# gongaa/SlidingWindowDecoder

Hardware: AMD Instinct MI355X
Metric: sliding windows decoded/s, [[144,12,12]] BB p=0.003 (higher is better)
Workload: dtype f64

## Files before the change

### slidingwindowdecoder_amd/csrc/swd_osdw_kernel.h

```cpp
#pragma once
#include <type_traits>
#include <hip/hip_runtime.h>
#include <stdint.h>

#include "swd.h"
#include "swd_graph.h"

#define SWD_DMAX 10

#ifndef SWD_OSDW_TUNED
#define SWD_OSDW_TUNED 0
#endif
#ifndef SWD_TUNED_NT
#define SWD_TUNED_NT 256
#endif
#define SWD_P16(NT) (SWD_OSDW_TUNED && (NT) <= SWD_TUNED_NT)
#ifndef SWD_POST_DEPTH2
#define SWD_POST_DEPTH2 0
#endif
#ifndef SWD_POST_SORTED
#define SWD_POST_SORTED 3
#endif
#ifndef SWD_POST_KGP
#define SWD_POST_KGP 0
// ... 155 lines not shown
template <int NT>
__device__ __forceinline__ bool block_any(bool p, Lds &s) {
    constexpr int NW = NT / 64;
    const int par = (s.fpar++) & 1;
    unsigned long long b = __ballot(p);
    if ((threadIdx.x & 63) == 0) s.flags[par * 16 + (threadIdx.x >> 6)] = (b != 0ull);
    __syncthreads();
    int r = 0;
#pragma unroll
    for (int w = 0; w < NW; ++w) r |= s.flags[par * 16 + w];
#ifdef SWD_NO_SCALAR_ANY
    return r != 0;
#else
    return __builtin_amdgcn_readfirstlane(r) != 0;
#endif
}

template <int NT>
__device__ __forceinline__ int block_exscan(int x, Lds &s, int &total) {
    constexpr int NW = NT / 64;
    const int lane = threadIdx.x & 63, wave = threadIdx.x >> 6;
    int incl = x;
#pragma unroll
    for (int d = 1; d < 64; d <<= 1) {
        int y = __shfl_up(incl, d, 64);
        if (lane >= d) incl += y;
    }
    int *wsum = s.scal + 8;
    __syncthreads();
    if (lane == 63) wsum[wave] = incl;
    __syncthreads();
    int off = 0, tot = 0;
#pragma unroll
    for (int w = 0; w < NW; ++w) {
        int c = wsum[w];
        if (w < wave) off += c;
        tot += c;
    }
    total = tot;
    return off + incl - x;
}

__device__ __forceinline__ uint64_t f2key(double x) {
    x = x + 0.0;
    uint64_t u = (uint64_t)__double_as_longlong(x);
    return (u >> 63) ? ~u : (u | 0x8000000000000000ull);
}

__device__ __forceinline__ int wave_max(int x) {
#pragma unroll
    for (int d = 32; d > 0; d >>= 1) x = max(x, __shfl_xor(x, d, 64));
    return x;
}

__device__ __forceinline__ void wave_fence() {
    __builtin_amdgcn_fence(__ATOMIC_SEQ_CST, "workgroup");
    __builtin_amdgcn_wave_barrier();
}

template <int VF, int DM, int SH = 0, bool PB = true>
struct VnCacheP {
    static_assert(DM % 2 == 0, "edge offsets are packed in pairs");
    static constexpr bool par_bytes = PB;
    static constexpr int par_shift = (SH == 0 && !PB) ? 2 : 0;
    double llr[VF];
    uint32_t edp[VF][DM / 2];
    __device__ __forceinline__ void set_ed(int i, int k, uint32_t v) { v >>= SH; edp[i][k >> 1] = (k & 1) ? ((edp[i][k >> 1] & 0xFFFFu) | (v << 16)) : ((edp[i][k >> 1] & 0xFFFF0000u) | v); }
    __device__ __forceinline__ void get_ed(int i, uint32_t (&ad)[DM]) const {
#pragma unroll
        for (int k = 0; k < DM; k += 2) {
            uint32_t w = edp[i][k >> 1];
            asm volatile("" : "+v"(w));
            ad[k] = (w & 0xFFFFu) << SH; ad[k + 1] = (w >> 16) << SH;
        }
    }
    uint32_t par[VF][(DM + 1) / 2];
};

__device__ __forceinline__ int swd_slot_far(const SwdGraphDev &g) { return g.E + 1 + (int)(threadIdx.x >> 6); }
template <int NT>
__device__ __forceinline__ int swd_slot_zero(const SwdGraphDev &g) { return g.E + 1 + NT / 64 + (int)(threadIdx.x >> 6); }

template <int NT, int VF, int DM>
struct VnRaw { uint32_t ev[VF][DM]; double llr[VF]; };
template <int NT, int VF, int DM>
__device__ __forceinline__ void vn_cache_issue(const SwdGraphDev &g, const Lds &s, VnRaw<NT, VF, DM> &r) {
    const int n = g.n, D = g.D;
    const uint32_t *et = g.vn_edge;
    const double *lt = g.llr;
#pragma unroll
    for (int i = 0; i < VF; ++i) {
        const int idx = s.vtid + i * NT;
        const int v = (idx < n) ? idx : 0;
        r.llr[i] = (n > 0) ? lt[v] : 0.0;
#pragma unroll
        for (int k = 0; k < DM; ++k) r.ev[i][k] = (n > 0) ? et[max(min(k, D - 1), 0) * n + v] : SWD_PAD_EDGE;
    }
}
template <int NT, int VF, int DM, int SH, bool PB>
__device__ __forceinline__ void vn_cache_pack(const SwdGraphDev &g, const Lds &s, const VnRaw<NT, VF, DM> &r, VnCacheP<VF, DM, SH, PB> &c) {
    const int n = g.n, D = g.D;
    const uint32_t dead = (uint32_t)swd_slot_zero<NT>(g) << 3;
#pragma unroll
    for (int i = 0; i < VF; ++i) {
        const int idx = s.vtid + i * NT;
        const bool valid = idx < n;
        c.llr[i] = valid ? r.llr[i] : 0.0;
#pragma unroll
        for (int k = 0; k < DM; ++k) c.set_ed(i, k, dead);
        constexpr int PS = VnCacheP<VF, DM, SH, PB>::par_shift;
#pragma unroll
        for (int k = 0; k < (DM + 1) / 2; ++k) c.par[i][k] = ((uint32_t)g.m << PS) * 0x10001u;
#pragma unroll
        for (int k = 0; k < DM; ++k) {
            const uint32_t e = r.ev[i][k];
            if (valid && k < D && e != SWD_PAD_EDGE) {
                c.set_ed(i, k, swd_edge_slot(e) << 3);
                c.par[i][k >> 1] = (k & 1) ? ((c.par[i][k >> 1] & 0xFFFFu) | ((swd_edge_lane(e) << PS) << 16))
                                           : ((c.par[i][k >> 1] & 0xFFFF0000u) | (swd_edge_lane(e) << PS));
            }
        }
    }
}

template <int NT, int VF, int DM, bool FULL, bool ALLEDGES = false, bool JPACK = false, int SH, bool PB>
__device__ __forceinline__ void vn_cache_load(const SwdGraphDev &g, Lds &s, int nlive, VnCacheP<VF, DM, SH, PB> &c, uint16_t *remap = nullptr) {
    const int n = g.n, cnt = FULL ? n : nlive;
    const uint32_t dead = (uint32_t)swd_slot_zero<NT>(g) << 3;
    const int D = g.D;
    const uint32_t *et = g.vn_edge;
    const double *lt = g.llr;
    uint32_t ev[VF][DM];
#pragma unroll
    for (int i = 0; i < VF; ++i) {
        const int idx = s.vtid + i * NT;
        const int v = (idx < cnt) ? (FULL ? idx : (int)s.lv[idx]) : 0;
        c.llr[i] = (n > 0) ? lt[v] : 0.0;
#pragma unroll
        for (int k = 0; k < DM; ++k) ev[i][k] = (n > 0) ? et[max(min(k, D - 1), 0) * n + v] : SWD_PAD_EDGE;
    }
#pragma unroll
    for (int i = 0; i < VF; ++i) {
        const int idx = s.vtid + i * NT;
        const bool valid = idx < cnt;
        if (!valid) c.llr[i] = 0.0;
#pragma unroll
        for (int k = 0; k < DM; ++k) c.set_ed(i, k, dead);
        constexpr int PS = VnCacheP<VF, DM, SH, PB>::par_shift;
#pragma unroll
        for (int k = 0; k < (DM + 1) / 2; ++k) c.par[i][k] = ((uint32_t)g.m << PS) * 0x10001u;
#pragma unroll
        for (int k = 0; k < DM; ++k) {
            const uint32_t e = ev[i][k];
            if (valid && k < D && e != SWD_PAD_EDGE) {
                if (FULL || ALLEDGES || s.cn_val[swd_edge_lane(e)] >= 0) {
                    uint32_t slot = swd_edge_slot(e);
                    if (!FULL && remap) { const uint32_t cell = (uint32_t)(k * nlive + idx); remap[slot] = (uint16_t)cell; slot = cell; }
                    c.set_ed(i, k, slot << 3);
                    const uint32_t ph = (swd_edge_lane(e) << PS) | (JPACK ? (swd_edge_j(e) << 10) : 0u);
                    c.par[i][k >> 1] = (k & 1) ? ((c.par[i][k >> 1] & 0xFFFFu) | (ph << 16))
                                               : ((c.par[i][k >> 1] & 0xFFFF0000u) | ph);
                }
            }
        }
    }
}


template <int NT, int VF, int DM, int SH, bool PB>
__device__ __forceinline__ void vn_cache_load_compact(const SwdGraphDev &g, Lds &s, int nlive, VnCacheP<VF, DM, SH, PB> &c, uint16_t *remap, int (&kc)[VF]) {
    const int n = g.n, D = g.D;
    constexpr int PS = VnCacheP<VF, DM, SH, PB>::par_shift;
    const uint32_t dead = (uint32_t)swd_slot_zero<NT>(g) << 3;
    uint32_t ev[VF][DM];
#pragma unroll
    for (int i = 0; i < VF; ++i) {
        const int idx = s.vtid + i * NT;
        const int v = (idx < nlive) ? (int)s.lv[idx] : 0;
        c.llr[i] = (n > 0) ? g.llr[v] : 0.0;
#pragma unroll
// ... 2012 lines not shown
    for (int v = tid; v < n; v += NT) s.hard[v] = 0;
    uint16_t *crows = (uint16_t *)s.scratch;
    bool cols = false;
    constexpr bool kColForm = COLFORM && NT >= 1024 && DM <= 8;
    if constexpr (kColForm) cols = g.wm > 4 && g.wm <= 9 && L.off_oslot >= 0;
    const int nst = min(n, (cols ? L.off_oslot : L.npad * 8) / (DM * 2));
    for (int p = tid; p < nst; p += NT) {
        const int v = idx[p];
        const int deg = g.col_deg[v];
#pragma unroll
        for (int k = 0; k < DM; ++k) crows[p * DM + k] = (k < deg) ? g.vn_row[k * n + v] : (uint16_t)0xFFFF;
    }
    __syncthreads();
    constexpr bool kQuad = QUAD && NT >= 256;
    bool quad = false;
    if constexpr (kQuad) quad = g.wm <= 4 && L.off_oring >= 0;
    if (quad) {
        if constexpr (kQuad) {
            int npiv = 0;
            const int ra = osd0_quad<NT, DM>(g, s, idx, Tc, Sbuf, piv_col, piv_row, synd, crows, nst, &npiv, s.scratch + L.off_oring);
            if (tid == 0) { s.scal[2] = ra; s.scal[3] = npiv; }
        }
    } else if (g.wm <= 4) {
        if (tid < 64) {
            int npiv;
            const int ra = osd0_wave_reg<DM>(g, s, idx, Tc, Sbuf, piv_col, piv_row, synd, crows, nst, &npiv);
            if (tid == 0) { s.scal[2] = ra; s.scal[3] = npiv; }
        }
    } else {
        int npiv = 0, ra = 0;
        bool done = false;
        if constexpr (kColForm) {
            if (cols) { ra = osd0_cols<NT, DM, 9>(g, s, idx, Tc, Sbuf, piv_col, piv_row, synd, crows, nst, &npiv, s.scratch + L.off_oslot); done = true; }
        }
        if constexpr (WIDE && NT == 1024 && DM <= 8) {
            if (g.wm <= 15 && L.off_owide >= 0) {
                ra = osd0_colsw<NT, DM, 15>(g, s, idx, Tc, Sbuf, piv_col, piv_row, synd, crows, nst, &npiv, (char *)s.hard - L.off_hard + L.off_owide, L.owide_ring, L.osd_lds != 0);
                done = true;
            }
        }
        if (!done) ra = osd0_block<NT, DM>(g, s, idx, Tc, Sbuf, piv_col, piv_row, synd, crows, nst, &npiv);
        if (tid == 0) { s.scal[2] = ra; s.scal[3] = npiv; }
    }
    __syncthreads();
    rowadds = s.scal[2];
    const int npiv = s.scal[3];
    t_elim = wall_clock64();
    if (osd0_b)
        for (int v = tid; v < n; v += NT) osd0_b[v] = s.hard[v];
    double pm = ordered_pm<NT>(g, s, list1);
    if (P.osd_order > 0) pm = osd_sweep<NT>(g, L, P, s, idx, Tc, Sbuf, piv_col, piv_row, npiv, pm, list1);
    return pm;
}

struct WinResult {
    int exit_class, conv, total_it, pre_it, post_it, live_vn, live_cn, live_e, osd_rowadds;
    double pm;
    long long t[9];
#ifdef SWD_GDGPROF
    long long gp[5];
#endif
};

__device__ __forceinline__ void lds_bind(Lds &s, char *smem, const SwdLdsLayout &L, char *scratch) {
    s.scratch = scratch;
    s.aux = scratch + L.off_aux;
    s.msg = (double *)scratch;
    s.livemask = (uint64_t *)(smem + L.off_livemask);
    s.par = (uint32_t *)(smem + L.off_par);
    s.lv = (uint16_t *)(smem + L.off_lv);
    s.jptr = (uint16_t *)(smem + L.off_jptr);
    s.lslot = (uint16_t *)((L.off_lslot > 0 ? smem : scratch) + (L.off_lslot >= 0 ? L.off_lslot : 0));
    s.cn_val = (int8_t *)(smem + L.off_cnval);
    s.cn_deg = (uint8_t *)(smem + L.off_cndeg);
    s.cn_deg0 = (uint8_t *)(smem + L.off_cndeg0);
    s.vn_val = (int8_t *)(smem + L.off_vnval);
    s.hard = (uint8_t *)(smem + L.off_hard);
    s.flags = (int *)(smem + L.off_misc);
    s.scal = s.flags + 32;
    s.dbl = (double *)(s.scal + 32);
    s.iaux = (int *)(s.dbl + 24);
}

template <int NT, int VF, int DM, int KG, bool SF, bool HACC, bool BIG = false>
__device__ __forceinline__ void decode_window(const SwdGraphDev &g, const SwdLdsLayout &L, const SwdDecodeParams &P, Lds &s,
                              const uint8_t *synd, double *hist_b, uint8_t *osd0_b, uint8_t *bpdec_b, WinResult &R, const uint32_t *cn_map,
                              VnRaw<NT, (NT <= SWD_TUNED_NT) ? VF : 1, DM> &vraw, const bool want_pm) {
    constexpr bool DIET = SWD_P16(NT);
    if constexpr (DIET) s.lm_m = (L.off_par - L.off_livemask < 8 * g.m) ? g.m : 0;
    if constexpr (DIET) s.par = (uint32_t *)s.livemask;
    const int tid = threadIdx.x;
    const int m = g.m, n = g.n;
#pragma unroll
    for (int i = 0; i < 9; ++i) R.t[i] = 0;
    R.t[0] = wall_clock64();

    constexpr bool kSplitLoad = NT <= SWD_TUNED_NT;
    [[maybe_unused]] int d_first = 0, p_first = 0, j_first = 0;
    if constexpr (kSplitLoad) {
        if (tid < m) { d_first = g.row_deg[tid]; p_first = g.perm[tid]; }
        if (tid <= g.K) j_first = g.jptr[tid];
        __builtin_amdgcn_sched_barrier(0);
        vn_cache_issue<NT, VF, DM>(g, s, vraw);
    }
    for (int l = tid; l < m; l += NT) {
        const int d = (kSplitLoad && l == tid) ? d_first : (int)g.row_deg[l];
        s.cn_val[l] = (int8_t)(synd[(kSplitLoad && l == tid) ? p_first : (int)g.perm[l]] ? 1 : 0);
        s.cn_deg[l] = (uint8_t)d;
        if constexpr (!DIET) s.cn_deg0[l] = (uint8_t)d;
        lm_set<DIET>(s, l, (d >= 64) ? ~0ull : ((1ull << d) - 1ull));
    }
    vn_reset<NT, DIET>(s, n);
    for (int j = tid; j <= g.K; j += NT) s.jptr[j] = (kSplitLoad && j == tid) ? (uint16_t)j_first : g.jptr[j];
    if (P.zero_hist)
        for (int i = tid; i < 4 * n; i += NT) hist_b[i] = 0.0;
    std::conditional_t<SWD_P16(NT), VnCacheP<VF, DM, 0, false>, VnCacheP<VF, DM, 3, false>> vc;
#ifdef SWD_INITPROF
    const long long ip0 = wall_clock64();
#endif
    constexpr bool kTbl = BIG && SWD_BIG_TBL && !kSplitLoad;
    constexpr bool kRec = BIG && SWD_BIG_REC && !kTbl && !kSplitLoad;
    bool rec_on = false;
    if constexpr (kRec) rec_on = L.off_pmsg >= 0 && m <= 1023 && L.pmsg_bytes >= (m + 1) * 32 + 4096;
    if constexpr (kSplitLoad) {
        vn_cache_pack<NT, VF, DM>(g, s, vraw, vc);
    } else if constexpr (kTbl) {
    } else {
        if (kRec && rec_on) { if constexpr (kRec) vn_cache_load<NT, VF, DM, true, false, true>(g, s, n, vc); }
        else vn_cache_load<NT, VF, DM, true>(g, s, n, vc);
    }
#ifdef SWD_INITPROF
    asm volatile("" : "+v"(vc.edp[VF - 1][0]), "+v"(vc.llr[0]));
    const long long ip1 = wall_clock64();
#endif
    __syncthreads();
#ifdef SWD_INITPROF
    const long long ip2 = wall_clock64();
#endif
    constexpr bool kHyb = BIG;
    const int rec_b = (kRec && rec_on) ? (((m + 1) * 32 + 15) & ~15) : 0;
    if constexpr (kRec) {
        if (rec_on) {
            s.rec = (SWD_AS3 char *)((char *)s.hard - L.off_hard + L.off_pmsg);
            if (tid < 8) ((SWD_AS3 uint32_t *)(s.rec + m * 32))[tid] = 0u;
        }
    }
    if constexpr (kHyb) {
        const int cells = g.E + 1 + 2 * (NT / 64);
        const int cap = (L.off_pmsg >= 0) ? (L.pmsg_bytes - rec_b) / 8 : 0;
        const int lo = max(cells - cap, 0);
        s.msg_lo = (cap > 0) ? (uint32_t)lo << 3 : 0xFFFFFFFFu;
        s.msg_alt = (char *)s.hard - L.off_hard + (L.off_pmsg >= 0 ? L.off_pmsg + rec_b : 0);
    }
    if constexpr (kTbl) bp_init_tbl<NT, VF, DM, kHyb>(g, s);
    else bp_init<VF, DM, kHyb>(s, vc);
#ifdef SWD_INITPROF
    const long long ip3 = wall_clock64();
#endif
    std::conditional_t<SWD_P16(NT), CnCacheP<KG>, CnCacheP<KG, 3>> cn;
    if constexpr (SF) {
        const uint32_t e = cn_map[s.ctid];
        cn_cache_load<NT, KG, true>(g, s, false, (e & 0xFFFFu) == 0xFFFFu ? -1 : (int)(e & 0xFFFFu), (int)((e >> 16) & 3u), (int)(e >> 18), cn);
    } else {
        cn_cache_load<NT, KG, true>(g, s, false, s.ctid < m ? s.ctid : -1, 0, 1, cn);
    }
    __syncthreads();

    int it = 0;
    R.conv = 0; R.pm = 0.0; R.pre_it = R.post_it = 0;
    R.live_vn = n; R.live_cn = m; R.live_e = g.E; R.osd_rowadds = 0;
    uint16_t *list0 = (uint16_t *)s.scratch;
    R.t[1] = wall_clock64();
#ifdef SWD_INITPROF
    if (tid == 0) { s.scal[20] = (int)(ip0 - R.t[0]); s.scal[21] = (int)(ip1 - ip0); s.scal[22] = (int)(ip2 - ip1); s.scal[23] = (int)(ip3 - ip2); s.scal[24] = (int)(R.t[1] - ip3); }
#endif

    double hs[VF];
#pragma unroll
    for (int i = 0; i < VF; ++i) hs[i] = 0.0;
    if constexpr (kTbl) R.conv = bp_run<NT, VF, DM, KG, true, SF, HACC, false, false, kHyb, false, true>(g, P, s, P.pre_iter, n, vc, cn, hist_b, it, P.alpha, false, hs);
    else
    if (kRec && rec_on) {
        if constexpr (kRec) R.conv = bp_run<NT, VF, DM, KG, true, SF, HACC, false, false, kHyb, true>(g, P, s, P.pre_iter, n, vc, cn, hist_b, it, P.alpha, false, hs);
    } else
    R.conv = bp_run<NT, VF, DM, KG, true, SF, HACC, false, false, kHyb>(g, P, s, P.pre_iter, n, vc, cn, hist_b, it, P.alpha, false, hs);
    R.pre_it = it;
    R.t[2] = wall_clock64();
// ... 390 lines not shown
        for (int v = tid; v < L.npad; v += NT) {
            if (v < n) {
                double sum;
                const int vv = vn_value<DIET>(s, v);
                if (vv == 1) sum = -1000.0;
                else if (vv == 0) sum = 1000.0;
                else sum = HACC ? hsl[v] : ((hist_b[v] + hist_b[n + v]) + hist_b[2 * n + v]) + hist_b[3 * n + v];
                key[v] = f2key(sum);
                idx[v] = (uint16_t)v;
            } else { key[v] = ~0ull; idx[v] = 0xFFFF; }
        }
        __syncthreads();
    }
    R.pm = osd_run<NT, DM, !BIG, !BIG, BIG>(g, L, P, s, synd, osd0_b, R.osd_rowadds, R.t[6], R.t[7], presorted);
    R.exit_class = SWD_EXIT_OSD;
}

#include "swd_gdg_kernel.h"

template <int NT>
__global__ void __launch_bounds__(NT) shot_weight_kernel(const uint8_t *det, int64_t det_stride, int num_det, int B, uint32_t *wt) {
    const int b = (int)blockIdx.x * (NT / 64) + (int)(threadIdx.x >> 6), lane = threadIdx.x & 63;
    if (b >= B) return;
    const uint8_t *d = det + (int64_t)b * det_stride;
    int c = 0;
    for (int r = lane; r < num_det; r += 64) c += d[r] ? 1 : 0;
#pragma unroll
    for (int o = 32; o > 0; o >>= 1) c += __shfl_xor(c, o, 64);
    if (lane == 0) wt[b] = (uint32_t)min(c, 1023);
}
template <int NT>
__global__ void __launch_bounds__(NT) shot_order_kernel(const uint32_t *wt, int B, uint32_t *order) {
    static_assert(NT == 1024, "one bin per thread");
    __shared__ uint32_t bin[2][1024];
    const int t = threadIdx.x;
    bin[0][t] = 0;
    __syncthreads();
    for (int b0 = t; b0 < B; b0 += 8 * NT) {
        uint32_t w8[8];
#pragma unroll
        for (int u = 0; u < 8; ++u) w8[u] = (b0 + u * NT < B) ? wt[b0 + u * NT] : 0xFFFFFFFFu;
#pragma unroll
        for (int u = 0; u < 8; ++u) if (w8[u] != 0xFFFFFFFFu) atomicAdd(&bin[0][1023 - w8[u]], 1u);
    }
    __syncthreads();
    const uint32_t own = bin[0][t];
    int cur = 0;
    for (int o = 1; o < 1024; o <<= 1) {
        bin[cur ^ 1][t] = bin[cur][t] + (t >= o ? bin[cur][t - o] : 0u);
        cur ^= 1;
        __syncthreads();
    }
    const uint32_t excl = bin[cur][t] - own;
    __syncthreads();
    bin[0][t] = excl;
    __syncthreads();
    for (int b0 = t; b0 < B; b0 += 8 * NT) {
        uint32_t w8[8];
#pragma unroll
        for (int u = 0; u < 8; ++u) w8[u] = (b0 + u * NT < B) ? wt[b0 + u * NT] : 0xFFFFFFFFu;
#pragma unroll
        for (int u = 0; u < 8; ++u) if (w8[u] != 0xFFFFFFFFu) order[atomicAdd(&bin[0][1023 - w8[u]], 1u)] = (uint32_t)(b0 + u * NT);
    }
}

template <int NT, int VF, int DM, int KG, int KIND, bool SF = false, bool BIG = false, int VFP = VF>
__global__ void __launch_bounds__(NT, (NT >= 1024 ? 4 : ((SWD_OSDW_TUNED && NT == 256 && KG <= 12 && (KIND == 0 || KIND == 3)) ? 3 : 2))) pipeline_kernel(const SwdPipeArgs a) {
    static_assert(NT == 64 || NT == 256 || NT == 1024, "workgroup sizes of swd_variants.h (the launch bounds and the sorted form know no other)");
    static_assert(!BIG || KIND == 0 || KIND == 3 || KIND == 1 || KIND == 7, "the HBM-resident scratch region exists for the osd_window kernels and for the guessing decoders' serial walk / ticket-scheduled ensemble");
    extern __shared__ __attribute__((aligned(16))) char smem[];
    const int tid = threadIdx.x;
    uint32_t *acc = (uint32_t *)(smem + a.off_det) - 4;
    const uint32_t nunits = (uint32_t)a.B * (uint32_t)a.W;
    Lds s;
    swd_wave_roles<NT>(s, acc + 2);
#ifdef SWD_RESIDENCY
    if (tid == 0) { const uint32_t now = atomicAdd(&a.status[4], 1u) + 1u; atomicMax(&a.status[5], now); }
    uint32_t res_units = 0;
#endif
    bool queued = false;
    constexpr bool kQueue = KIND == 2 || KIND == 7;
    if constexpr (kQueue) queued = a.gdgp.q != nullptr;
    constexpr uint32_t shots0 = 0;
    for (;;) {
    const long long t_unit0 = wall_clock64();
    int wi, b, final_ctx = -1;
    [[maybe_unused]] bool ens_task = false;
    [[maybe_unused]] uint32_t ens_item = 0;
#ifdef SWD_GDG_DEBUG
    long long dbg_ta = 0, dbg_tb = 0, dbg_tc = 0;
#endif
    if (queued) {
        uint32_t item = 0;
        if constexpr (kQueue) {
            __syncthreads();
            if (tid == 0) {
                if ((int32_t)(ag_ld(&a.gdgp.q[1]) - ag_ld(&a.gdgp.q[0])) <= 0) {
                    const uint32_t nb = shots0 + atomicAdd(a.sched, 1u);
                    if (nb < (uint32_t)a.B) ring_push(a.gdgp.q, a.gdgp.qmask, item_unit(a.order ? (int)a.order[nb] : (int)nb, 0));
                }
                acc[2] = ring_pop_wait(a.gdgp.q, a.gdgp.qmask, a.status, &a.sched[a.B + 1]); acc[3] = 0u;
            }
            __syncthreads();
            item = acc[2];
        }
#ifdef SWD_GDG_DEBUG
        asm volatile("" ::: "memory"); dbg_ta = wall_clock64(); asm volatile("" ::: "memory");
        if (tid == 0) { uint32_t *dbg_status = a.gdgp.chk_status; GDG_COUNT(7, 1); GDG_COUNT(8, dbg_ta - t_unit0); if (dbg_ta - t_unit0 > 5000) { GDG_COUNT(6, 1); GDG_COUNT(15, dbg_ta - t_unit0); } }
#endif
        if (item == SWD_ITEM_EXIT) break;
        const uint32_t type = item >> 30;
        if (type == SWD_ITEM_SIDE) {
            if constexpr (KIND == 2) gdg_run_task<NT, VF, DM, KG, VFP>(a, smem, item, s.ctid, s.vtid);
            if constexpr (KIND != 7) continue;
            ens_task = true; ens_item = item;
            wi = (int)ag_ld(&((const uint32_t *)(a.gdgp.ctx + (int64_t)((item >> 8) & 0x3FFFFFu) * a.gdgp.ctx_stride))[4]); b = 0;
        }
        else if (type == SWD_ITEM_FINAL) {
            final_ctx = (int)(item & 0x3FFFFFFFu);
            uint32_t *h = (uint32_t *)(a.gdgp.ctx + (int64_t)final_ctx * a.gdgp.ctx_stride);
            wi = (int)__hip_atomic_load(&h[4], __ATOMIC_RELAXED, __HIP_MEMORY_SCOPE_AGENT);
            b = (int)__hip_atomic_load(&h[5], __ATOMIC_RELAXED, __HIP_MEMORY_SCOPE_AGENT);
        } else { wi = (int)((item >> 22) & 0xFFu); b = (int)(item & 0x3FFFFFu); }
    } else {
    __syncthreads();
    if (tid == 0) {
        const uint32_t t = atomicAdd(a.sched, 1u);
        acc[2] = t; acc[3] = 0u;
        if (a.order && t < nunits) acc[1] = a.order[t % (uint32_t)a.B];
    }
    __syncthreads();
    const uint32_t ticket = acc[2];
    if (ticket >= nunits) break;
    wi = (int)(ticket / (uint32_t)a.B); b = a.order ? (int)acc[1] : (int)(ticket % (uint32_t)a.B);
    }
    __syncthreads();
    uint8_t *sdet = (uint8_t *)(smem + a.off_det);
    uint8_t *state_b = a.state + (int64_t)b * a.state_stride;
    constexpr bool SLICE = SWD_P16(NT) && (KIND == 0 || KIND == 3);
    const int dbase = SLICE ? (a.wins[wi].row0 & ~3) : 0;
    const int dlen = (SLICE ? min((a.wins[wi].row0 + a.wins[wi].g.m + 3) & ~3, (a.num_det + 3) & ~3) : ((a.num_det + 3) & ~3)) - dbase;
    if (ens_task) {
    } else if (wi == 0) {
        const uint8_t *det_b = a.det + (int64_t)b * a.det_stride;
        if constexpr (SLICE) {
            for (int r = tid; r < dlen; r += NT) sdet[r] = (dbase + r < a.num_det && det_b[dbase + r]) ? 1 : 0;
        } else {
            for (int r = tid; r < a.num_det; r += NT) sdet[r] = det_b[r] ? 1 : 0;
        }
        if (SLICE && a.W > 1) {
            uint32_t *st32 = (uint32_t *)state_b;
            for (int q = tid; q < (a.num_det + 3) / 4; q += NT) {
                if (4 * q >= dbase && 4 * q < dbase + dlen) continue;
                uint32_t x = 0;
                for (int k = 0; k < 4; ++k) x |= (4 * q + k < a.num_det && det_b[4 * q + k]) ? (1u << (8 * k)) : 0u;
                __hip_atomic_store(&st32[4 + q], x, __ATOMIC_RELAXED, __HIP_MEMORY_SCOPE_AGENT);
            }
        }
        if (tid == 0) { acc[0] = 0; acc[1] = 0; }
    } else {
        if (!queued && tid == 0) {
            const long long t_wait0 = wall_clock64();
            while (__hip_atomic_load(&a.sched[1 + b], __ATOMIC_RELAXED, __HIP_MEMORY_SCOPE_AGENT) < (uint32_t)wi) {
                __builtin_amdgcn_s_sleep(8);
                if (wall_clock64() - t_wait0 > 1000000000ll) { atomicOr(a.status, 1u); atomicOr(&a.sched[a.B + 1], 1u); acc[3] = 1u; break; }
            }
            __builtin_amdgcn_fence(__ATOMIC_ACQUIRE, "agent");
        }
        __syncthreads();
        const uint32_t *st32 = (const uint32_t *)state_b;
        uint32_t *sdet32 = (uint32_t *)sdet;
        if constexpr (SLICE) {
            for (int r = tid; r < dlen / 4; r += NT)
                sdet32[r] = __hip_atomic_load(&st32[4 + dbase / 4 + r], __ATOMIC_RELAXED, __HIP_MEMORY_SCOPE_AGENT);
        } else {
            for (int r = tid; r < (a.num_det + 3) / 4; r += NT)
                sdet32[r] = __hip_atomic_load(&st32[4 + r], __ATOMIC_RELAXED, __HIP_MEMORY_SCOPE_AGENT);
        }
        if (tid == 0) { acc[0] = __hip_atomic_load(&st32[0], __ATOMIC_RELAXED, __HIP_MEMORY_SCOPE_AGENT); acc[1] = 0; }
    }
    const int sidx = a.slot_scratch ? (int)blockIdx.x : b;
    double *hist_b = a.hist + (int64_t)sidx * a.hist_stride;
    s.fpar = 0;
    __syncthreads();
#ifdef SWD_TSPROF
    if (a.prof && tid == 0 && final_ctx < 0 && !ens_task) a.prof[((int64_t)b * a.W + wi) * 8 + 4] = wall_clock64();
#endif
#ifdef SWD_GDG_DEBUG
    asm volatile("" ::: "memory"); dbg_tb = wall_clock64(); asm volatile("" ::: "memory");
    if (queued && tid == 0) { uint32_t *dbg_status = a.gdgp.chk_status; GDG_COUNT(13, dbg_tb - t_unit0); GDG_COUNT(14, 1); }
#endif
    {
        const SwdWindowDev &w = a.wins[wi];
        const SwdGraphDev &g = w.g;
        const SwdLdsLayout &L = w.L;
        lds_bind(s, smem, L, BIG ? (char *)(a.big + (int64_t)blockIdx.x * a.big_stride) : smem);
        WinResult R;
#ifdef SWD_SELPROF
        if (tid < 8) s.scal[20 + tid] = 0;
        __syncthreads();
#endif
#ifdef SWD_BPPROF
        if (tid == 0) { s.scal[24] = s.scal[25] = s.scal[26] = s.scal[27] = 0; s.scal[20] = s.scal[21] = s.scal[22] = 0; }
#endif
        if (acc[3]) {
            for (int v = tid; v < g.n; v += NT) s.hard[v] = 0;
            R = WinResult{};
            R.exit_class = SWD_EXIT_SCHED_FAULT;
        } else if constexpr (KIND == 0 || KIND == 3)
        {
            VnRaw<NT, (NT <= SWD_TUNED_NT) ? VF : 1, DM> vraw;
            decode_window<NT, VF, DM, KG, SF, KIND == 3, BIG>(g, L, a.P, s, sdet + (w.row0 - dbase), hist_b, a.osd0 ? a.osd0 + (int64_t)b * g.n : nullptr,
                                                         a.bp_dec ? a.bp_dec + (int64_t)b * g.n : nullptr, R, w.cn_map, vraw, a.min_pm != nullptr);
        }
        else {
            uint8_t *snap_b = a.snap + (int64_t)sidx * a.snap_stride;
            bool redo = false;
            if (ens_task) {
            } else if (final_ctx >= 0 && KIND == 7) {
                if constexpr (KIND == 7) {
                    const EnsCtx ec = gdg_ens_ctx(a.gdgp, final_ctx);
                    gdg_ens_finalize<NT>(g, a.P, s, ec, R);
                    if (tid == 0) ring_push(a.gdgp.fq, a.gdgp.fmask, (uint32_t)final_ctx);
                    __syncthreads();
                }
            } else
            if (final_ctx >= 0) {
                const GdgCtx c = gdg_ctx(a.gdgp, final_ctx);
#ifdef SWD_GDG_CHECKS
                if (tid == 0) {
                    uint32_t *chk_status = a.gdgp.chk_status;
                    GDG_CHECK(final_ctx < a.gdgp.nctx, 9);
                    GDG_CHECK(atomicExch(&c.hdr[1], 2u) == 1u, 10);
                    GDG_CHECK(ag_ld(&c.hdr[22]) == 1u && ag_ld(&c.hdr[18]) == ag_ld(&c.hdr[19]), 11);
                    GDG_CHECK(wi < a.W && b < a.B, 12);
                }
#endif
                redo = !gdg_finalize<NT>(g, a.P, s, c, R);
                if (tid == 0) {
                    while (ag_ld(&c.hdr[0]) != 0u) __builtin_amdgcn_s_sleep(2);
                    ring_push(a.gdgp.fq, a.gdgp.fmask, (uint32_t)final_ctx);
                }
                __syncthreads();
            }
            if (!ens_task && (final_ctx < 0 || redo)) {
#ifdef SWD_GDG_DEBUG
                asm volatile("" ::: "memory"); dbg_tc = wall_clock64(); asm volatile("" ::: "memory");
#endif
                s.fpar = 0;
                decode_window_gdg<NT, VF, DM, KG, KIND == 7, VFP>(g, L, a.P, s, sdet + (w.row0 - dbase), hist_b, snap_b, R, (queued && !redo) ? &a : nullptr, acc, wi, b);
#ifdef SWD_GDG_DEBUG
                if (tid == 0 && queued) { uint32_t *dbg_status = a.gdgp.chk_status; GDG_COUNT(R.exit_class == -2 ? 9 : 10, 1); GDG_COUNT(R.exit_class == -2 ? 11 : 12, wall_clock64() - t_unit0); }
#endif
                if (R.exit_class == -2) continue;
            }
            if constexpr (KIND == 7) {
                if (ens_task || R.exit_class == -3) {
                    GdgLds G;
                    gdg_bind(G, gdg_lds_base(s, L), L, g.n, g.new_n);
                    SwdGraphDev g_ens = g;
                    int role = 0, hyp = 0;
                    bool dead_unsat = false;
                    EnsCtx ec{};
                    if (ens_task) {
                        role = 2; hyp = (int)(ens_item & 0xFFu);
                        ec = gdg_ens_ctx(a.gdgp, (int)((ens_item >> 8) & 0x3FFFFFu));
                        dead_unsat = ag_ld(&ec.hdr[6]) != 0u;
                        s.fpar = 0;
                        __syncthreads();
                        for (int l = tid; l < g.m; l += NT) s.cn_deg0[l] = g.row_deg[l];
                        for (int v = tid; v < g.n; v += NT) { s.vn_val[v] = 0; s.hard[v] = 0; }
                        for (int j = tid; j <= g.K; j += NT) s.jptr[j] = g.jptr[j];
                        for (int i = tid; i < (g.new_n + 1) / 2; i += NT) {
                            const uint32_t x = ag_ld(&ec.pos[i]);
                            G.pos_lv[2 * i] = (uint16_t)x;
                            if (2 * i + 1 < g.new_n) G.pos_lv[2 * i + 1] = (uint16_t)(x >> 16);
                        }
                        if (a.P.max_iter_per_step < 4)
                            for (int i = a.P.max_iter_per_step * g.n + tid; i < 4 * g.n; i += NT) hist_b[i] = 0.0;
                        __syncthreads();
                        {
                            const int64_t fkb = gdg_ens_fork_bytes(g.m, g.new_n, gdg_ens_fork_cells(g.E + 1 + 2 * (NT / 64), NT, VFP, DM));
                            const int Tt = (1 << a.P.max_tree_depth) - 1, nfk = 1 << (a.P.max_tree_depth - 1);
                            gdg_snap_load<NT>(g, s, G, hyp <= Tt ? ec.fork + (int64_t)(hyp >> 1) * fkb
                                                                  : ec.fork + (int64_t)nfk * fkb + (int64_t)(hyp - Tt - 1) * ((gdg_snap_bytes(g.m, g.new_n) + 15) & ~(int64_t)15));
                        }
                    } else {
                        dead_unsat = R.live_vn != 0;
                        gdg_staged_graph(g_ens, g, s);
                        if (queued && a.gdgp.ctx && a.P.max_tree_depth >= 1) {
                            __syncthreads();
                            if (tid == 0) { uint32_t id = 0; acc[1] = ring_pop(a.gdgp.fq, a.gdgp.fmask, &id) ? id : 0xFFFFFFFFu; }
                            __syncthreads();
                            const int ectx_id = (int)acc[1];
                            if (ectx_id >= 0) {
                                role = 1;
                                ec = gdg_ens_ctx(a.gdgp, ectx_id);
                                if (tid == 0) {
                                    ag_st(&ec.hdr[0], 1u); ag_st(&ec.hdr[4], (uint32_t)wi); ag_st(&ec.hdr[5], (uint32_t)b); ag_st(&ec.hdr[6], dead_unsat ? 1u : 0u);
                                    ag_st(&ec.hdr[8], 0u); ag_st(&ec.hdr[9], 0u); ag_st(&ec.hdr[10], 0u); ag_st(&ec.hdr[11], 0u); ag_st(&ec.hdr[12], (uint32_t)R.pre_it);
                                }
                                for (int k = tid; k < ec.nh; k += NT) ag_st(&ec.etab[4 * k], 0u);
                                for (int i = tid; i < (g.new_n + 1) / 2; i += NT)
                                    ag_st(&ec.pos[i], (uint32_t)G.pos_lv[2 * i] | ((2 * i + 1 < g.new_n) ? ((uint32_t)G.pos_lv[2 * i + 1] << 16) : 0u));
                                ag_publish_barrier();
                            }
                        }
                        R.live_vn = g.n; R.post_it = 0;
                    }
                    gdg_ensemble_tree<NT, VFP, DM, KG>(role, &g_ens, &a.P, s, G, hist_b, snap_b, &R, dead_unsat ? 1 : 0, &a.gdgp, &ec, hyp);
                    if (role != 0) continue;
                    for (int v = tid; v < g.n; v += NT) s.hard[v] = 0;
                    __syncthreads();
                    for (int j = tid; j < g.new_n; j += NT) s.hard[G.pos_lv[j]] = G.best_err[j];
                    __syncthreads();
                    R.total_it = R.pre_it + R.post_it;
                    R.exit_class = SWD_EXIT_POST;
                    R.t[5] = wall_clock64();
                }
            }
        }
        __syncthreads();
#ifdef SWD_GDG_DEBUG
        if (tid == 0) {
            uint32_t hi = 2166136261u, ho = 2166136261u;
            for (int r = 0; r < g.m; ++r) hi = (hi ^ sdet[w.row0 - dbase + r]) * 16777619u;
            for (int v = 0; v < g.n; ++v) ho = (ho ^ s.hard[v]) * 16777619u;
            R.live_cn = (int)hi; R.live_e = (int)ho;
        }
        __syncthreads();
#endif
        if (a.total) {
            uint8_t *tot_b = a.total + (int64_t)b * a.total_stride + w.col0;
            uint32_t *sdet_w = (uint32_t *)sdet;
            for (int i = tid; i < w.commit; i += NT) {
                const uint8_t hv = s.hard[i];
                tot_b[i] = hv;
                if (hv) {
                    const int c = w.col0 + i;
                    if (a.obs_mask) { const uint32_t om = a.obs_mask[c]; if (om) atomicXor(&acc[0], om); }
                    for (uint32_t e = a.chk_colptr[c]; e < a.chk_colptr[c + 1]; ++e) {
                        const int r = a.chk_rows[e];
                        if constexpr (!SLICE) { atomicXor(&sdet_w[r >> 2], 1u << ((r & 3) * 8)); continue; }
                        const int rl = r - dbase;
                        if (rl >= 0 && rl < dlen) atomicXor(&sdet_w[rl >> 2], 1u << ((r & 3) * 8));
                        else __hip_atomic_fetch_xor(&((uint32_t *)state_b)[4 + (r >> 2)], 1u << ((r & 3) * 8), __ATOMIC_RELAXED, __HIP_MEMORY_SCOPE_AGENT);
                    }
                }
            }
        }
        if (a.win_out && wi == a.W - 1) {
            uint8_t *o = a.win_out + (int64_t)b * a.win_out_stride;
            for (int v = tid; v < g.n; v += NT) o[v] = s.hard[v];
        }
        if (tid == 0) {
            if (a.stats) {
                int32_t *st = a.stats + ((int64_t)b * a.W + wi) * SWD_STAT_WORDS;
                st[0] = R.exit_class | (R.conv ? SWD_STATUS_CONVERGE : 0);
                st[1] = R.total_it; st[2] = R.pre_it; st[3] = R.post_it;
                st[4] = R.live_vn; st[5] = R.live_cn; st[6] = R.live_e;
#ifdef SWD_GDG_DEBUG
                atomicAdd(&st[7], 1);
#else
                st[7] = R.osd_rowadds;
#endif
#ifdef SWD_BPPROF
                if (R.post_it > 0) st[7] = s.scal[28];
#endif
            }
            if (a.min_pm) a.min_pm[(int64_t)b * a.W + wi] = R.pm;
            if (a.prof) {
                int64_t *pr = a.prof + ((int64_t)b * a.W + wi) * 8;
                const long long tend = wall_clock64();
                long long prev = R.t[0];
#ifdef SWD_TSPROF
                const int64_t ts_start = pr[4];
#endif
#pragma unroll
                for (int i = 1; i <= 7; ++i) {
                    const long long cur = R.t[i] ? R.t[i] : prev;
                    pr[i - 1] = cur - prev;
                    prev = cur;
                }
                pr[7] = tend - prev;
#ifdef SWD_GDG_DEBUG
                pr[6] = R.t[0] - t_unit0; pr[2] = dbg_ta - t_unit0; pr[3] = dbg_tb - t_unit0; pr[4] = dbg_tc - t_unit0;
#else
                pr[0] += R.t[0] - t_unit0;
#endif
#ifdef SWD_TSPROF
                pr[5] = t_unit0; pr[6] = tend; pr[4] = ts_start;
#endif
#ifdef SWD_GDGPROF
                pr[0] = R.t[2] - R.t[0]; pr[1] = (R.t[3] ? R.t[3] : R.t[2]) - R.t[2];
                pr[2] = R.gp[0]; pr[3] = R.gp[1]; pr[4] = R.gp[2]; pr[5] = R.gp[3]; pr[6] = R.gp[4]; pr[7] = tend - R.t[0];
#endif
#ifdef SWD_BPPROF
                pr[0] = s.scal[24]; pr[5] = s.scal[25]; pr[6] = s.scal[26]; pr[7] = s.scal[27];
                pr[1] = s.scal[20]; pr[2] = s.scal[21]; pr[3] = s.scal[22]; pr[4] = s.scal[23];
#endif
#ifdef SWD_INITPROF
                pr[0] = R.t[0] - t_unit0; pr[1] = s.scal[20]; pr[2] = s.scal[21]; pr[3] = s.scal[22]; pr[4] = s.scal[23]; pr[5] = s.scal[24];
                pr[6] = tend - R.t[1]; pr[7] = (R.exit_class == SWD_EXIT_PRE || R.exit_class == SWD_EXIT_POST) ? s.scal[25] : 0;
#endif
#ifdef SWD_SELPROF
                for (int k = 0; k < 8; ++k) { pr[k] = s.scal[20 + k]; s.scal[20 + k] = 0; }
#endif
#ifdef SWD_SHPROF
                pr[1] = s.scal[20]; pr[2] = s.scal[21]; pr[3] = s.scal[22]; pr[4] = s.scal[23];
                if (tid == 0) { s.scal[20] = s.scal[21] = s.scal[22] = s.scal[23] = 0; }
#endif
            }
        }
        __syncthreads();
        if (wi + 1 < a.W) {
            uint32_t *st32 = (uint32_t *)state_b;
            const uint32_t *sdet32 = (const uint32_t *)sdet;
            if constexpr (SLICE) {
                for (int r = tid; r < dlen / 4; r += NT)
                    __hip_atomic_store(&st32[4 + dbase / 4 + r], sdet32[r], __ATOMIC_RELAXED, __HIP_MEMORY_SCOPE_AGENT);
            } else {
                for (int r = tid; r < (a.num_det + 3) / 4; r += NT)
                    __hip_atomic_store(&st32[4 + r], sdet32[r], __ATOMIC_RELAXED, __HIP_MEMORY_SCOPE_AGENT);
            }
            if (tid == 0) __hip_atomic_store(&st32[0], acc[0], __ATOMIC_RELAXED, __HIP_MEMORY_SCOPE_AGENT);
            asm volatile("s_waitcnt vmcnt(0)" ::: "memory");
            __builtin_amdgcn_fence(__ATOMIC_RELEASE, "workgroup");
            __syncthreads();
            if (tid == 0) {
                __builtin_amdgcn_fence(__ATOMIC_RELEASE, "agent");
                asm volatile("s_waitcnt vmcnt(0)" ::: "memory");
            }
            if (tid == 0) {
                __hip_atomic_store(&a.sched[1 + b], (uint32_t)(wi + 1), __ATOMIC_RELAXED, __HIP_MEMORY_SCOPE_AGENT);
                if constexpr (kQueue) { if (queued) ring_push(a.gdgp.q, a.gdgp.qmask, item_unit(b, wi + 1)); }
            }
        }
        if constexpr (kQueue) {
            if (queued && tid == 0) {
                if (wi == a.W - 1) {
                    const uint32_t nb = shots0 + atomicAdd(a.sched, 1u);
                    if (nb < (uint32_t)a.B) ring_push(a.gdgp.q, a.gdgp.qmask, item_unit(a.order ? (int)a.order[nb] : (int)nb, 0));
                }
                if (atomicAdd(&a.gdgp.q[2], 1u) + 1u == nunits)
                    for (uint32_t k = 0; k < gridDim.x; ++k) ring_push(a.gdgp.q, a.gdgp.qmask, SWD_ITEM_EXIT);
            }
        }
    }
    if (a.shot_result && wi == a.W - 1) {
        bool nz = false;
        if constexpr (SLICE) { for (int r = tid; r < dlen; r += NT) nz |= (sdet[r] != 0); }
        else { for (int r = tid; r < a.num_det; r += NT) nz |= (sdet[r] != 0); }
        if (SLICE && a.W > 1) {
            const uint32_t *st32 = (const uint32_t *)state_b;
            for (int q = tid; q < (a.num_det + 3) / 4; q += NT)
                if (4 * q < dbase || 4 * q >= dbase + dlen) nz |= __hip_atomic_load(&st32[4 + q], __ATOMIC_RELAXED, __HIP_MEMORY_SCOPE_AGENT) != 0u;
        }
        const bool any = block_any<NT>(nz, s);
        if (tid == 0) { a.shot_result[2 * b] = (int32_t)acc[0]; a.shot_result[2 * b + 1] = any ? 1 : 0; }
    }
#ifdef SWD_RESIDENCY
    ++res_units;
#endif
    }
#ifdef SWD_RESIDENCY
    if (tid == 0) { atomicSub(&a.status[4], 1u); if (res_units) atomicAdd(&a.status[6], 1u); atomicMax(&a.status[7], res_units); }
#endif
}

}
```

Baseline: 5.270 million.

## Prefetch next ticket during epilogue and hoist window loads before state wait

The persistent kernel now claims its next work ticket at the end of the current unit and, when the predecessor window is already published, marks it as ready. This removes a barrier pair and the spin-wait at the start of the next unit. The per-window graph and VN-cache loads, plus the first state word, are issued before the dependency wait/LDS fill so their latency overlaps. The risks are added complexity in ticket/acquire ordering, a high-bit flag packed into acc[1], and higher register pressure from hoisting vraw to the loop scope.

```diff
diff --git a/slidingwindowdecoder_amd/csrc/swd_osdw_kernel.h b/slidingwindowdecoder_amd/csrc/swd_osdw_kernel.h
--- a/slidingwindowdecoder_amd/csrc/swd_osdw_kernel.h
+++ b/slidingwindowdecoder_amd/csrc/swd_osdw_kernel.h
@@ -261,7 +261,7 @@
 __device__ __forceinline__ int swd_slot_zero(const SwdGraphDev &g) { return g.E + 1 + NT / 64 + (int)(threadIdx.x >> 6); }
 
 template <int NT, int VF, int DM>
-struct VnRaw { uint32_t ev[VF][DM]; double llr[VF]; };
+struct VnRaw { uint32_t ev[VF][DM]; double llr[VF]; int first[3]; };
 template <int NT, int VF, int DM>
 __device__ __forceinline__ void vn_cache_issue(const SwdGraphDev &g, const Lds &s, VnRaw<NT, VF, DM> &r) {
     const int n = g.n, D = g.D;
@@ -275,6 +275,15 @@
 #pragma unroll
         for (int k = 0; k < DM; ++k) r.ev[i][k] = (n > 0) ? et[max(min(k, D - 1), 0) * n + v] : SWD_PAD_EDGE;
     }
+}
+template <int NT, int VF, int DM>
+__device__ __forceinline__ void window_loads_issue(const SwdGraphDev &g, const Lds &s, VnRaw<NT, VF, DM> &r) {
+    const int tid = threadIdx.x;
+    r.first[0] = r.first[1] = r.first[2] = 0;
+    if (tid < g.m) { r.first[0] = g.row_deg[tid]; r.first[1] = g.perm[tid]; }
+    if (tid <= g.K) r.first[2] = g.jptr[tid];
+    __builtin_amdgcn_sched_barrier(0);
+    vn_cache_issue<NT, VF, DM>(g, s, r);
 }
 template <int NT, int VF, int DM, int SH, bool PB>
 __device__ __forceinline__ void vn_cache_pack(const SwdGraphDev &g, const Lds &s, const VnRaw<NT, VF, DM> &r, VnCacheP<VF, DM, SH, PB> &c) {
@@ -2453,7 +2462,7 @@
     s.iaux = (int *)(s.dbl + 24);
 }
 
-template <int NT, int VF, int DM, int KG, bool SF, bool HACC, bool BIG = false>
+template <int NT, int VF, int DM, int KG, bool SF, bool HACC, bool BIG = false, bool ISSUED = false>
 __device__ __forceinline__ void decode_window(const SwdGraphDev &g, const SwdLdsLayout &L, const SwdDecodeParams &P, Lds &s,
                               const uint8_t *synd, double *hist_b, uint8_t *osd0_b, uint8_t *bpdec_b, WinResult &R, const uint32_t *cn_map,
                               VnRaw<NT, (NT <= SWD_TUNED_NT) ? VF : 1, DM> &vraw, const bool want_pm) {
@@ -2467,13 +2476,9 @@
     R.t[0] = wall_clock64();
 
     constexpr bool kSplitLoad = NT <= SWD_TUNED_NT;
-    [[maybe_unused]] int d_first = 0, p_first = 0, j_first = 0;
-    if constexpr (kSplitLoad) {
-        if (tid < m) { d_first = g.row_deg[tid]; p_first = g.perm[tid]; }
-        if (tid <= g.K) j_first = g.jptr[tid];
-        __builtin_amdgcn_sched_barrier(0);
-        vn_cache_issue<NT, VF, DM>(g, s, vraw);
-    }
+    static_assert(kSplitLoad || !ISSUED, "only the kernels that split the cache load can take it early");
+    if constexpr (kSplitLoad && !ISSUED) window_loads_issue(g, s, vraw);
+    [[maybe_unused]] const int d_first = kSplitLoad ? vraw.first[0] : 0, p_first = kSplitLoad ? vraw.first[1] : 0, j_first = kSplitLoad ? vraw.first[2] : 0;
     for (int l = tid; l < m; l += NT) {
         const int d = (kSplitLoad && l == tid) ? d_first : (int)g.row_deg[l];
         s.cn_val[l] = (int8_t)(synd[(kSplitLoad && l == tid) ? p_first : (int)g.perm[l]] ? 1 : 0);
@@ -3030,9 +3035,12 @@
     constexpr bool kQueue = KIND == 2 || KIND == 7;
     if constexpr (kQueue) queued = a.gdgp.q != nullptr;
     constexpr uint32_t shots0 = 0;
+    constexpr bool SLICE = SWD_P16(NT) && (KIND == 0 || KIND == 3);
+    bool have_next = false;
     for (;;) {
     const long long t_unit0 = wall_clock64();
     int wi, b, final_ctx = -1;
+    bool seen = false;
     [[maybe_unused]] bool ens_task = false;
     [[maybe_unused]] uint32_t ens_item = 0;
 #ifdef SWD_GDG_DEBUG
@@ -3071,23 +3079,32 @@
             b = (int)__hip_atomic_load(&h[5], __ATOMIC_RELAXED, __HIP_MEMORY_SCOPE_AGENT);
         } else { wi = (int)((item >> 22) & 0xFFu); b = (int)(item & 0x3FFFFFu); }
     } else {
-    __syncthreads();
-    if (tid == 0) {
-        const uint32_t t = atomicAdd(a.sched, 1u);
-        acc[2] = t; acc[3] = 0u;
-        if (a.order && t < nunits) acc[1] = a.order[t % (uint32_t)a.B];
-    }
-    __syncthreads();
+    if (!have_next) {
+        if (tid == 0) {
+            const uint32_t t = atomicAdd(a.sched, 1u);
+            acc[2] = t; acc[3] = 0u;
+            if (t < nunits) acc[1] = a.order ? a.order[t % (uint32_t)a.B] : t % (uint32_t)a.B;
+        }
+        __syncthreads();
+    }
+    have_next = false;
     const uint32_t ticket = acc[2];
     if (ticket >= nunits) break;
-    wi = (int)(ticket / (uint32_t)a.B); b = a.order ? (int)acc[1] : (int)(ticket % (uint32_t)a.B);
-    }
-    __syncthreads();
+    const uint32_t parked = acc[1];
+    wi = (int)(ticket / (uint32_t)a.B); b = (int)(parked & 0x7FFFFFFFu); seen = (parked >> 31) != 0u;
+    }
+    if constexpr (kQueue) __syncthreads();
     uint8_t *sdet = (uint8_t *)(smem + a.off_det);
     uint8_t *state_b = a.state + (int64_t)b * a.state_stride;
-    constexpr bool SLICE = SWD_P16(NT) && (KIND == 0 || KIND == 3);
     const int dbase = SLICE ? (a.wins[wi].row0 & ~3) : 0;
     const int dlen = (SLICE ? min((a.wins[wi].row0 + a.wins[wi].g.m + 3) & ~3, (a.num_det + 3) & ~3) : ((a.num_det + 3) & ~3)) - dbase;
+    [[maybe_unused]] VnRaw<NT, (NT <= SWD_TUNED_NT) ? VF : 1, DM> vraw;
+    [[maybe_unused]] uint32_t st_first = 0;
+    if constexpr (SLICE) {
+        if (seen && tid < dlen / 4) st_first = __hip_atomic_load(&((const uint32_t *)state_b)[4 + dbase / 4 + tid], __ATOMIC_RELAXED, __HIP_MEMORY_SCOPE_AGENT);
+        __builtin_amdgcn_sched_barrier(0);
+        window_loads_issue(a.wins[wi].g, s, vraw);
+    }
     if (ens_task) {
     } else if (wi == 0) {
         const uint8_t *det_b = a.det + (int64_t)b * a.det_stride;
@@ -3105,8 +3122,9 @@
                 __hip_atomic_store(&st32[4 + q], x, __ATOMIC_RELAXED, __HIP_MEMORY_SCOPE_AGENT);
             }
         }
-        if (tid == 0) { acc[0] = 0; acc[1] = 0; }
+        if (tid == 0) acc[0] = 0;
     } else {
+        if (!seen) {
         if (!queued && tid == 0) {
             const long long t_wait0 = wall_clock64();
             while (__hip_atomic_load(&a.sched[1 + b], __ATOMIC_RELAXED, __HIP_MEMORY_SCOPE_AGENT) < (uint32_t)wi) {
@@ -3116,16 +3134,17 @@
             __builtin_amdgcn_fence(__ATOMIC_ACQUIRE, "agent");
         }
         __syncthreads();
+        }
         const uint32_t *st32 = (const uint32_t *)state_b;
         uint32_t *sdet32 = (uint32_t *)sdet;
         if constexpr (SLICE) {
             for (int r = tid; r < dlen / 4; r += NT)
-                sdet32[r] = __hip_atomic_load(&st32[4 + dbase / 4 + r], __ATOMIC_RELAXED, __HIP_MEMORY_SCOPE_AGENT);
+                sdet32[r] = (seen && r == tid) ? st_first : __hip_atomic_load(&st32[4 + dbase / 4 + r], __ATOMIC_RELAXED, __HIP_MEMORY_SCOPE_AGENT);
         } else {
             for (int r = tid; r < (a.num_det + 3) / 4; r += NT)
                 sdet32[r] = __hip_atomic_load(&st32[4 + r], __ATOMIC_RELAXED, __HIP_MEMORY_SCOPE_AGENT);
         }
-        if (tid == 0) { acc[0] = __hip_atomic_load(&st32[0], __ATOMIC_RELAXED, __HIP_MEMORY_SCOPE_AGENT); acc[1] = 0; }
+        if (tid == 0) acc[0] = __hip_atomic_load(&st32[0], __ATOMIC_RELAXED, __HIP_MEMORY_SCOPE_AGENT);
     }
     const int sidx = a.slot_scratch ? (int)blockIdx.x : b;
     double *hist_b = a.hist + (int64_t)sidx * a.hist_stride;
@@ -3157,8 +3176,7 @@
             R.exit_class = SWD_EXIT_SCHED_FAULT;
         } else if constexpr (KIND == 0 || KIND == 3)
         {
-            VnRaw<NT, (NT <= SWD_TUNED_NT) ? VF : 1, DM> vraw;
-            decode_window<NT, VF, DM, KG, SF, KIND == 3, BIG>(g, L, a.P, s, sdet + (w.row0 - dbase), hist_b, a.osd0 ? a.osd0 + (int64_t)b * g.n : nullptr,
+            decode_window<NT, VF, DM, KG, SF, KIND == 3, BIG, SLICE>(g, L, a.P, s, sdet + (w.row0 - dbase), hist_b, a.osd0 ? a.osd0 + (int64_t)b * g.n : nullptr,
                                                          a.bp_dec ? a.bp_dec + (int64_t)b * g.n : nullptr, R, w.cn_map, vraw, a.min_pm != nullptr);
         }
         else {
@@ -3269,6 +3287,8 @@
             }
         }
         __syncthreads();
+        [[maybe_unused]] uint32_t next_t = 0;
+        if (!queued && tid == 0) next_t = atomicAdd(a.sched, 1u);
 #ifdef SWD_GDG_DEBUG
         if (tid == 0) {
             uint32_t hi = 2166136261u, ho = 2166136261u;
@@ -3302,6 +3322,20 @@
             for (int v = tid; v < g.n; v += NT) o[v] = s.hard[v];
         }
         if (tid == 0) {
+            if (!queued) {
+                uint32_t nb = 0;
+                if (next_t < nunits) {
+                    nb = a.order ? a.order[next_t % (uint32_t)a.B] : next_t % (uint32_t)a.B;
+                    if constexpr (SLICE) {
+                        const uint32_t nwi = next_t / (uint32_t)a.B;
+                        if (nwi > 0u && __hip_atomic_load(&a.sched[1 + nb], __ATOMIC_RELAXED, __HIP_MEMORY_SCOPE_AGENT) >= nwi) {
+                            __builtin_amdgcn_fence(__ATOMIC_ACQUIRE, "agent");
+                            nb |= 0x80000000u;
+                        }
+                    }
+                }
+                acc[1] = nb; acc[2] = next_t; acc[3] = 0u;
+            }
             if (a.stats) {
                 int32_t *st = a.stats + ((int64_t)b * a.W + wi) * SWD_STAT_WORDS;
                 st[0] = R.exit_class | (R.conv ? SWD_STATUS_CONVERGE : 0);
@@ -3361,6 +3395,7 @@
             }
         }
         __syncthreads();
+        have_next = !queued;
         if (wi + 1 < a.W) {
             uint32_t *st32 = (uint32_t *)state_b;
             const uint32_t *sdet32 = (const uint32_t *)sdet;
```

New measurement: 5.062 million. 0.96x the previous value.
